# guanjq/targetdiff

Measured on AMD Instinct MI355X. Metric: ligands/sec (1000-step sampling, 100 samples/pocket) at 1/2/4/8 MI355X, higher is better.
Workload: dtype f32

## Files before the change

targetdiff_amd/csrc/edge16.hip:

```cpp
#include <type_traits>

#include "td_device.h"
#include "td_internal.h"

typedef float floatx4_t __attribute__((ext_vector_type(4)));

__device__ __forceinline__ floatx4_t td_mfma16(float a, float b, floatx4_t c) {
    return __builtin_amdgcn_mfma_f32_16x16x4f32(a, b, c, 0, 0, 0);
}

typedef _Float16 half8_16 __attribute__((ext_vector_type(8)));
__device__ __forceinline__ floatx4_t td_mfma16h(uint4 a, uint4 b, floatx4_t c) {
    return __builtin_amdgcn_mfma_f32_16x16x32_f16(__builtin_bit_cast(half8_16, a), __builtin_bit_cast(half8_16, b), c, 0, 0, 0);
}
__device__ __forceinline__ void td_split_h2(float x, float y, unsigned &h1, unsigned &h2) {
    h1 = __builtin_bit_cast(unsigned, __builtin_amdgcn_cvt_pkrtz(x, y));
    asm("v_fma_mixlo_f16 %0, %1, -1.0, %2 op_sel_hi:[1,0,0]\n\t"
        "v_fma_mixhi_f16 %0, %1, -1.0, %3 op_sel:[1,0,0] op_sel_hi:[1,0,0]"
        : "=&v"(h2) : "v"(h1), "v"(x), "v"(y));
}
constexpr float TD_Z_SCALE = 32768.0f;
__device__ __forceinline__ void td_split_h2_scaled_x4(const float (&x)[4], const float (&y)[4], unsigned (&h1)[4], unsigned (&h2)[4]) {
    const float S = TD_Z_SCALE;
    asm("v_fma_mixlo_f16 %0, %8, %16, 0\n\t"
// ... 1945 lines not shown
            a.h[(size_t)i * TD_H + nout + 4] = hres1 + o1;
        }
    }
    if (a.trace) {
        td_trace_wave_end(a.trace, lane);
        __syncthreads();
        if (tid == 0) a.trace[8 * blockIdx.x + 1] = __builtin_amdgcn_s_memrealtime();
    }
}

constexpr int TD_GATE_WGS = 1024;
constexpr int G16_WAVES = 4;
constexpr int G16Q_U4 = e16q_cs_u4<1>();
constexpr size_t G16_LDS_BYTES = (size_t)G16Q_U4 * 16 + (size_t)3 * TD_H * sizeof(float);

__global__ __launch_bounds__(G16_WAVES * 64) void edge_gate16_kernel(TdGate gt, const float4 *__restrict__ x4,
                                                                     const int32_t *__restrict__ nbr, int64_t N,
                                                                     const int32_t *__restrict__ rows,
                                                                     const int32_t *__restrict__ count_ptr,
                                                                     const int32_t *__restrict__ chunk_node, float *__restrict__ ew) {
    extern __shared__ __attribute__((aligned(16))) float lds[];
    const uint4 *Rp = reinterpret_cast<const uint4 *>(lds);
    float *B0 = lds + G16Q_U4 * 4, *BET = B0 + TD_H, *W3 = BET + TD_H;
    const int tid = threadIdx.x, lane = tid & 63, wid = tid >> 6;
    const int lo = lane & 15, g = lane >> 4;
    {
        td_stage_pk4<1>(gt.R16q, lds, 1, tid, G16_WAVES * 64);
        for (int t = tid; t < 3 * TD_H; t += G16_WAVES * 64) {
            const int n = t & (TD_H - 1);
            B0[t] = t < TD_H ? gt.b0[n] : (t < 2 * TD_H ? gt.beta[n] : gt.w3[n]);
        }
    }
    float offj[5];
#pragma unroll
    for (int j = 0; j < 5; ++j) offj[j] = gt.offsets[5 * g + j];
    __syncthreads();
    int64_t begin, end;
    td_node_range16(N, count_ptr, begin, end);
    const float c2 = gt.coeff * TD_LOG2E;

    for (int64_t it = begin + wid; it < end; it += G16_WAVES) {
        const int64_t row = rows ? (int64_t)rows[it] : it;
        const int64_t i = chunk_node ? (int64_t)chunk_node[row] : row;
        const float4 xi = x4[i];
        int jn[2];
        jn[0] = nbr[row * TD_K + lo];
        jn[1] = nbr[row * TD_K + 16 + lo];
        floatx4_t acc[2][8];
        uint4 bq[2][4];
        bool valid[2];
#pragma unroll
        for (int eb = 0; eb < 2; ++eb) {
            valid[eb] = jn[eb] >= 0;
            const float4 xj = x4[valid[eb] ? jn[eb] : (int)i];
            const float rx = xi.x - xj.x, ry = xi.y - xj.y, rz = xi.z - xj.z;
            const float dist = td_sqrt_d2(rx * rx + ry * ry + rz * rz);
            float gv[5];
#pragma unroll
            for (int j = 0; j < 5; ++j) {
                const float u = dist - offj[j];
                gv[j] = __builtin_amdgcn_exp2f(c2 * (u * u));
            }
            td_pk4_bquads(gv, 0u, bq[eb]);
#pragma unroll
            for (int hb = 0; hb < 8; ++hb) {
                const float4 b = *reinterpret_cast<const float4 *>(B0 + 16 * hb + 4 * g);
                acc[eb][hb][0] = b.x; acc[eb][hb][1] = b.y; acc[eb][hb][2] = b.z; acc[eb][hb][3] = b.w;
            }
        }
        td_pk4_tiles<1, 1, 2>(Rp + lane, lane, bq, acc);
        td_ln_relu16<2>(BET, g, acc, TdLn{gt.ln_c1, gt.ln_c2});
#pragma unroll
        for (int eb = 0; eb < 2; ++eb) {
            float part = 0.f;
#pragma unroll
            for (int hb = 0; hb < 8; ++hb) {
                const float4 w = *reinterpret_cast<const float4 *>(W3 + 16 * hb + 4 * g);
                part = fmaf(acc[eb][hb][0], w.x, part); part = fmaf(acc[eb][hb][1], w.y, part);
                part = fmaf(acc[eb][hb][2], w.z, part); part = fmaf(acc[eb][hb][3], w.w, part);
            }
            const float logit = td_sum_groups(part) + gt.b3;
            if (g == 0) ew[row * TD_K + 16 * eb + lo] = valid[eb] ? 1.0f / (1.0f + expf(-logit)) : 0.f;
        }
    }
}

template __global__ void edge_key16_kernel<false, K16S_WAVES, 0, 2, true, 0, 1>(Args16);
template __global__ void edge_key16_kernel<false, K16S_WAVES, 0, 2, true, 0, 0>(Args16);
template __global__ void edge_key16_kernel<false, K16S_WAVES, 0, 2, true, 2, 1>(Args16);
template __global__ void edge_key16_kernel<false, K16S_WAVES, 0, 2, true, 2, 0>(Args16);
template __global__ void edge_key16_kernel<false, K16S_WAVES, 0, 2, true, 1, 1>(Args16);
template __global__ void edge_key16_kernel<false, K16S_WAVES, 0, 2, true, 1, 0>(Args16);
template __global__ void edge_key16_kernel<false, K16S_WAVES, 0, 1, true, 0, 1>(Args16);
template __global__ void edge_key16_kernel<false, K16S_WAVES, 0, 1, true, 0, 0>(Args16);
template __global__ void edge_key16_kernel<false, K16S_WAVES, 0, 1, true, 2, 1>(Args16);
template __global__ void edge_key16_kernel<false, K16S_WAVES, 0, 1, true, 1, 1>(Args16);
template __global__ void edge_key16_kernel<false, K16S_WAVES, 1, 1, true, 0, 1>(Args16);
template __global__ void edge_key16_kernel<false, K16S_WAVES, 1, 1, true, 0, 0>(Args16);
template __global__ void edge_key16_kernel<false, K16S_WAVES, 1, 0, true, 0, 1>(Args16);
template __global__ void edge_key16_kernel<false, K16S_WAVES, 1, 0, true, 0, 0>(Args16);
// ... 219 lines not shown
    const bool split = mlp_k.use_split && mlp_v.use_split;
    if (cptr) {
        if (f16_first) return td_launch<edge_h2x16_chunked_kernel<1>>(grid, block, h2x16_lds_bytes<true>(), s, ar);
        return td_launch<edge_h2x16_chunked_kernel<0>>(grid, block, h2x16_lds_bytes<true>(), s, ar);
    }
    if (split && f16_first) return td_launch<edge_h2x16_kernel<true, 1>>(grid, block, h2x16_lds_bytes<true>(), s, ar);
    if (split) return td_launch<edge_h2x16_kernel<true, 0>>(grid, block, h2x16_lds_bytes<true>(), s, ar);
    return td_launch<edge_h2x16_kernel<false, 0>>(grid, block, h2x16_lds_bytes<false>(), s, ar);
}

int td_launch_gate16(const TdGate &g, const float4 *x4, const int32_t *nbr, int64_t N, const int32_t *rows,
                     const int32_t *count_ptr, float *ew, hipStream_t s, const int32_t *chunk_node) {
    if (N == 0) return TD_OK;
    int64_t G = (N + G16_WAVES - 1) / G16_WAVES;
    if (G > TD_GATE_WGS) G = TD_GATE_WGS;
    return td_launch<edge_gate16_kernel>(dim3((unsigned)G), dim3(G16_WAVES * 64), G16_LDS_BYTES, s, g, x4, nbr, N, rows, count_ptr, chunk_node, ew);
}
```

targetdiff_amd/csrc/graph.hip:

```cpp
#include "td_device.h"
#include "td_internal.h"

__global__ void graph_ptr_kernel(const int64_t *__restrict__ batch, int64_t N, int64_t B, int32_t *__restrict__ ptr) {
    int64_t i = (int64_t)blockIdx.x * blockDim.x + threadIdx.x;
    if (N == 0) {
        if (i <= B) ptr[i] = 0;
        return;
    }
    if (i >= N) return;
    int64_t b = batch[i];
    int64_t prev = (i == 0) ? -1 : batch[i - 1];
    for (int64_t g = prev + 1; g <= b && g <= B; ++g) ptr[g] = (int32_t)i;
    if (i == N - 1)
        for (int64_t g = b + 1; g <= B; ++g) ptr[g] = (int32_t)N;
}

int td_launch_graph_ptr(const int64_t *batch, int64_t N, int64_t B, int32_t *ptr, hipStream_t s) {
    int64_t n = N > B + 1 ? N : B + 1;
    graph_ptr_kernel<<<dim3((unsigned)((n + 255) / 256)), dim3(256), 0, s>>>(batch, N, B, ptr);
    TD_CHECK_HIP(hipGetLastError());
    return TD_OK;
}

__global__ void node_gid_kernel(const int32_t *__restrict__ ptr, int64_t N, int B, int32_t *__restrict__ gid) {
// ... 147 lines not shown
int td_launch_knn_rows(const float4 *x4, const int32_t *node_ptr, const int32_t *gid, const int32_t *rows, int64_t count,
                       int max_graph_nodes, int32_t *nbr, hipStream_t s, int k) {
    return launch_knn_t<false>(x4, node_ptr, gid, rows, count, max_graph_nodes, k, nbr, nullptr, s);
}

int td_launch_knn_static(const float4 *x4, const int32_t *node_ptr, const int32_t *gid, const int32_t *rows, int64_t count,
                         int max_graph_nodes, int32_t *nbr, unsigned long long *skeys, hipStream_t s, int k) {
    return launch_knn_t<true>(x4, node_ptr, gid, rows, count, max_graph_nodes, k, nbr, skeys, s);
}

struct TdMergeArgs {
    const float4 *x4; const int32_t *ptr, *pptr, *gid, *prot_rows; int64_t Np;
    const unsigned long long *skeys; const int32_t *snbr; const float *h0, *h1s, *ews; int32_t *nbr; float *h, *ew;
    uint8_t *clean, *flags2; int k;
    const int32_t *cgraph, *cbase;
};
__device__ __forceinline__ void knn_merge_body(unsigned bid, const TdMergeArgs &ma) {
    const float4 *__restrict__ x4 = ma.x4;
    const int32_t *__restrict__ ptr = ma.ptr, *__restrict__ pptr = ma.pptr, *__restrict__ gid = ma.gid, *__restrict__ prot_rows = ma.prot_rows;
    const int64_t Np = ma.Np;
    const unsigned long long *__restrict__ skeys = ma.skeys;
    const int32_t *__restrict__ snbr = ma.snbr;
    const float *__restrict__ h0 = ma.h0, *__restrict__ h1s = ma.h1s, *__restrict__ ews = ma.ews;
    int32_t *__restrict__ nbr = ma.nbr;
    float *__restrict__ h = ma.h, *__restrict__ ew = ma.ew;
    uint8_t *__restrict__ clean = ma.clean, *__restrict__ flags2 = ma.flags2;
    const int k = ma.k;
    const int lane = threadIdx.x & 63;
    const int64_t qi = (int64_t)bid * 4 + (threadIdx.x >> 6);
    if (qi >= Np) return;
// ... 1 lines not shown
    const int g = gid[i];
    const int lbeg = ptr[g] + (pptr[g + 1] - pptr[g]), lend = ptr[g + 1];
    const float4 xi = x4[i];
    int64_t c = i;
    int rebase = 0;
    if (ma.cgraph) {
        rebase = ptr[g] - ptr[ma.cgraph[g]];
        c = (int64_t)ma.cbase[g] + (i - ptr[g]);
    }
    unsigned long long ks = lane < TD_K ? skeys[c * TD_K + lane] : TD_KEY_MAX;
    if (ks != TD_KEY_MAX) ks += (unsigned long long)(unsigned)rebase;
    const unsigned long long thr = __shfl(ks, k - 1);
    unsigned long long kl[2] = {TD_KEY_MAX, TD_KEY_MAX};
    bool closer = false;
    bool overflow = lend - lbeg > 128;
#pragma unroll
    for (int u = 0; u < 2; ++u) {
        const int j = lbeg + lane + 64 * u;
        if (j < lend) {
            const float4 xj = x4[j];
            const float d2 = td_dist2(xj.x - xi.x, xj.y - xi.y, xj.z - xi.z);
            kl[u] = ((unsigned long long)__float_as_uint(d2) << 32) | (unsigned)j;
            closer |= kl[u] < thr;
        }
    }
    bool is_clean = !overflow && __ballot(closer) == 0ull;
    if (!is_clean && !overflow) {
        const bool c0 = kl[0] < thr, c1 = kl[1] < thr;
        const unsigned long long m0 = __ballot(c0), m1 = __ballot(c1);
        const int n_static = __popcll(__ballot(lane < TD_K && ks != TD_KEY_MAX));
// ... 1 lines not shown
        bool lig_in = false;
#pragma unroll
        for (int u = 0; u < 2; ++u) {
            unsigned long long mm = u ? m1 : m0;
            while (mm) {
                const int src = __builtin_amdgcn_readfirstlane(__ffsll((long long)mm) - 1);
                mm &= mm - 1;
                const unsigned clo = __builtin_amdgcn_readlane((int)(unsigned)kl[u], src);
                const unsigned chi = __builtin_amdgcn_readlane((int)(unsigned)(kl[u] >> 32), src);
                const unsigned long long ck = ((unsigned long long)chi << 32) | clo;
                if (lane < TD_K && ck < ks) ++shift;
                const int rank = __popcll(__ballot(lane < TD_K && ks < ck)) + __popcll(__ballot(c0 && kl[0] < ck)) +
                                 __popcll(__ballot(c1 && kl[1] < ck));
                if (rank < k) {
                    lig_in = true;
                    if (lane == 0) nbr[i * TD_K + rank] = (int32_t)clo;
                }
            }
        }
        const int total = n_static + __popcll(m0) + __popcll(m1);
        if (lane < TD_K) {
            const int pos = lane + shift;
            if (ks != TD_KEY_MAX && pos < k) nbr[i * TD_K + pos] = (int32_t)(unsigned)(ks & 0xffffffffull);
            if (lane >= (total < k ? total : k)) nbr[i * TD_K + lane] = -1;
        }
        is_clean = !lig_in;
    } else if (!is_clean) {
        unsigned long long best = ks;
        for (int base = lbeg; base < lend; base += 128) {
            if (base != lbeg) {
#pragma unroll
                for (int u = 0; u < 2; ++u) {
                    const int j = base + lane + 64 * u;
                    kl[u] = TD_KEY_MAX;
                    if (j < lend) {
                        const float4 xj = x4[j];
                        const float d2 = td_dist2(xj.x - xi.x, xj.y - xi.y, xj.z - xi.z);
                        kl[u] = ((unsigned long long)__float_as_uint(d2) << 32) | (unsigned)j;
                    }
                }
            }
// ... 13 lines not shown
            best = out;
        }
        if (lane < TD_K) nbr[i * TD_K + lane] = (best == TD_KEY_MAX || lane >= k) ? -1 : (int32_t)(unsigned)(best & 0xffffffffull);
        const bool lig_in = lane < k && best != TD_KEY_MAX && (int)(unsigned)(best & 0xffffffffull) >= lbeg;
        is_clean = __ballot(lig_in) == 0ull;
    } else if (lane < TD_K) {
        const int32_t sj = snbr[c * TD_K + lane];
        nbr[i * TD_K + lane] = sj >= 0 ? sj + rebase : -1;
    }
    const float2 hv = *reinterpret_cast<const float2 *>((is_clean ? h1s : h0) + c * TD_H + 2 * lane);
    *reinterpret_cast<float2 *>(h + i * TD_H + 2 * lane) = hv;
    if (is_clean && lane < TD_K) ew[i * TD_K + lane] = ews[c * TD_K + lane];
    if (lane == 0) {
        clean[i] = is_clean ? 1 : 0;
        if (flags2) flags2[i] = 0;
    }
}

__global__ __launch_bounds__(256) void knn_merge_kernel(TdMergeArgs ma) { knn_merge_body(blockIdx.x, ma); }

template <int CH>
__global__ __launch_bounds__(256) void knn_step_kernel(TdMergeArgs ma, unsigned GB, const int32_t *__restrict__ lig_rows, int64_t Nl,
                                                       int32_t *__restrict__ nbr) {
    if (blockIdx.x < GB) knn_body<CH, false>(blockIdx.x, ma.x4, ma.ptr, ma.gid, lig_rows, Nl, ma.k, nbr, nullptr);
    else knn_merge_body(blockIdx.x - GB, ma);
}

int td_launch_knn_merge(const float4 *x4, const int32_t *node_ptr, const int32_t *pptr, const int32_t *gid,
                        const int32_t *prot_rows, int64_t Np, const unsigned long long *skeys, const int32_t *snbr,
                        const float *h0, const float *h1s, const float *ews, int32_t *nbr, float *h, float *ew,
                        uint8_t *clean, uint8_t *flags2, hipStream_t s, int k, const int32_t *lig_rows, int64_t Nl,
                        int max_graph_nodes, const int32_t *cgraph, const int32_t *cbase) {
    const TdMergeArgs ma{x4, node_ptr, pptr, gid, prot_rows, Np, skeys, snbr, h0, h1s, ews, nbr, h, ew, clean, flags2, k, cgraph, cbase};
    const unsigned GA = (unsigned)((Np + 3) / 4), GB = lig_rows ? (unsigned)((Nl + 3) / 4) : 0u;
    if (GA + GB == 0) return TD_OK;
    if (GB == 0) {
        knn_merge_kernel<<<dim3(GA), dim3(256), 0, s>>>(ma);
    } else {
        const dim3 grid(GA + GB), block(256);
        if (max_graph_nodes > 0 && max_graph_nodes <= 256) knn_step_kernel<4><<<grid, block, 0, s>>>(ma, GB, lig_rows, Nl, nbr);
        else if (max_graph_nodes > 0 && max_graph_nodes <= 384) knn_step_kernel<6><<<grid, block, 0, s>>>(ma, GB, lig_rows, Nl, nbr);
        else if (max_graph_nodes <= 704) knn_step_kernel<11><<<grid, block, 0, s>>>(ma, GB, lig_rows, Nl, nbr);
        else knn_step_kernel<17><<<grid, block, 0, s>>>(ma, GB, lig_rows, Nl, nbr);
    }
    TD_CHECK_HIP(hipGetLastError());
    return TD_OK;
}

// ... 325 lines not shown
        int32_t *c = counter[0];
#pragma unroll
        for (int q = 1; q < L; ++q) c = l == q ? counter[q] : c;
        s_base[l] = (total && c) ? atomicAdd(c, total) : 0;
    }
    __syncthreads();
#pragma unroll
    for (int l = 0; l < L; ++l) {
        int before = 0;
        for (int w = 0; w < wave; ++w) before += s_cnt[l][w];
        slot[l] = s_base[l] + before + __popcll(m[l] & below);
    }
    __syncthreads();
}

constexpr int TD_LISTS_THREADS = 1024;

template <bool CHUNKED>
__global__ __launch_bounds__(TD_LISTS_THREADS) void step_lists_kernel(const uint8_t *__restrict__ clean, const float4 *__restrict__ x4,
                                                                      const int32_t *__restrict__ nbr, const int32_t *__restrict__ node_ptr,
                                                                      const int32_t *__restrict__ cptr, const int32_t *__restrict__ chunk_node,
                                                                      int64_t N, int cap, TdStepLists out) {
    constexpr int T = TD_LISTS_THREADS, RPT = T / TD_K;
    extern __shared__ uint8_t s_flags[];
    uint8_t *dirty = s_flags, *reach = s_flags + cap, *level = s_flags + 2 * cap, *lig = s_flags + 3 * cap;
    const int n0 = node_ptr[blockIdx.x], n = node_ptr[blockIdx.x + 1] - n0;
    const int tid = threadIdx.x, e = tid & 31, r0 = tid >> 5;
    const int t0 = CHUNKED ? cptr[n0] : n0, nt = CHUNKED ? cptr[n0 + n] - t0 : n;
    for (int a = tid; a < n; a += T) {
        const bool l = x4[n0 + a].w > 0.5f;
// ... 46 lines not shown
        bool flag[TD_STEP_LISTS];
        flag[0] = in && dirty[a];
        flag[1] = in && out.reach_rows && reach[a];
        flag[2] = in && out.reach_rows && !reach[a];
#pragma unroll
        for (int k = 0; k < TD_HOP_LEVELS; ++k) flag[3 + k] = k < out.levels && lv != 0 && lv <= k + 1;
        int slot[TD_STEP_LISTS];
        td_block_slots_each<TD_STEP_LISTS, T / 64>(flag, counters, slot);
        const int32_t i = n0 + a;
        if (flag[0]) out.dirty_rows[slot[0]] = i;
        if (flag[1]) out.reach_rows[slot[1]] = i;
        if (flag[2]) out.rest_rows[slot[2]] = i;
#pragma unroll
        for (int k = 0; k < TD_HOP_LEVELS; ++k)
            if (flag[3 + k]) out.level_rows[(size_t)k * N + slot[3 + k]] = i;
    }
    if (CHUNKED && out.dirty_chunks) {
        int32_t *const cc[1] = {out.dirty_chunk_count};
        for (int base = 0; base < nt; base += T) {
            const int t = base + tid;
            const bool flag[1] = {t < nt && dirty[dst_of(t < nt ? t : 0)]};
            int slot[1];
            td_block_slots_each<1, T / 64>(flag, cc, slot);
            if (flag[0]) out.dirty_chunks[slot[0]] = t0 + t;
        }
    }
}

int td_launch_step_lists(const uint8_t *clean, const float4 *x4, const int32_t *nbr, const int32_t *node_ptr, int64_t N,
                         int64_t B, int max_nodes, const TdStepLists &out, hipStream_t s, const int32_t *cptr,
// ... 8 lines not shown
        step_lists_kernel<false><<<dim3((unsigned)B), dim3(TD_LISTS_THREADS), bytes, s>>>(clean, x4, nbr, node_ptr, nullptr, nullptr, N, cap, out);
    TD_CHECK_HIP(hipGetLastError());
    return TD_OK;
}

__global__ __launch_bounds__(128) void ligand_update_kernel(const float *__restrict__ lpos, const int64_t *__restrict__ lv,
                                                            const int32_t *__restrict__ lig_node, int64_t Nl, int C,
                                                            const float *__restrict__ WlT, const float *__restrict__ bl,
                                                            float *__restrict__ h, float4 *__restrict__ x4, TdStepReset rs,
                                                            const float *__restrict__ gbias, const int32_t *__restrict__ gid) {
    const int n = threadIdx.x;
    if (blockIdx.x == 0) {
        if (rs.c0 && n < rs.n0) rs.c0[n] = 0;
        if (rs.c1 && n < rs.n1) rs.c1[n] = 0;
        if (rs.c2 && n < rs.n2) rs.c2[n] = 0;
    }
    const int64_t a0 = (int64_t)blockIdx.x * TD_COMPOSE_ATOMS;
    const float bias = bl[n];
    for (int a = 0; a < TD_COMPOSE_ATOMS; ++a) {
        const int64_t at = a0 + a;
        if (at >= Nl) break;
        const int64_t p = lig_node[at];
        int v = (int)lv[at];
        v = v < 0 ? 0 : (v >= C ? C - 1 : v);
        h[p * TD_H + n] = (gbias ? WlT[v * TD_H + n] + gbias[(size_t)gid[p] * TD_H + n] : WlT[v * TD_H + n]) + bias;
        if (n == 0) {
            x4[p] = make_float4(lpos[3 * at], lpos[3 * at + 1], lpos[3 * at + 2], 1.f);
            if (rs.flags2) rs.flags2[p] = 0;
        }
    }
// ... 307 lines not shown
```

targetdiff_amd/csrc/pack.cpp:

```cpp
#include <algorithm>
#include <atomic>
#include <cmath>
#include <cstdarg>
#include <cstdio>
#include <cstdlib>
#include <cstring>
#include <mutex>
#include <new>
#include <vector>

#include "td_device.h"
#include "td_internal.h"
#include "td_api.h"

using namespace tdapi;

namespace tdapi {



struct FoldedMlp {
    std::vector<float> w0, b0, g, b, w3, b3v;
    const float *b3;
    float ln_c1 = 1.f / 128.f, ln_c2 = 1e-5f;
// ... 353 lines not shown
enum OptKind { OPT_FLAG, OPT_CLAMPED, OPT_RANGED };
struct OptRow { const char *name; int TdOptions::*field; OptKind kind; int lo, hi; };
const OptRow OPTIONS[] = {
    {"h2x_fused", &TdOptions::h2x_fused, OPT_FLAG, 0, 1},
    {"node_proj_split", &TdOptions::node_proj_split, OPT_FLAG, 0, 1},
    {"node_proj_bpipe", &TdOptions::node_proj_bpipe, OPT_FLAG, 0, 1},
    {"node_proj_async", &TdOptions::node_proj_async, OPT_FLAG, 0, 1},
    {"edge_key_split", &TdOptions::edge_key_split, OPT_FLAG, 0, 1},
    {"edge_first_layer_f16", &TdOptions::edge_first_layer_f16, OPT_FLAG, 0, 1},
    {"edge_second_layer_f16", &TdOptions::edge_second_layer_f16, OPT_FLAG, 0, 1},
    {"edge_row_dealing", &TdOptions::edge_row_dealing, OPT_CLAMPED, 0, 2},
    {"session_hop_levels", &TdOptions::session_hop_levels, OPT_RANGED, 1, TD_HOP_LEVELS},
    {"session_forward_reach", &TdOptions::session_forward_reach, OPT_FLAG, 0, 1},
    {"session_step_lists", &TdOptions::session_step_lists, OPT_FLAG, 0, 1},
    {"session_share_pockets", &TdOptions::session_share_pockets, OPT_FLAG, 0, 1},
};
struct ReadOnlyRow { const char *name; int td_model::*field; };
const ReadOnlyRow READ_ONLY[] = {{"fold_dead_units", &td_model::fold_dead_units}, {"fold_fp32_mlps", &td_model::fold_fp32_mlps}};

template <class Row, size_t N>
const Row *find_row(const Row (&rows)[N], const char *name) {
    for (const Row &r : rows)
        if (strcmp(r.name, name) == 0) return &r;
    return nullptr;
}

void apply_options(td_model *m) {
    const TdOptions &o = m->opt;
    m->gate.use_split = o.edge_key_split != 0;
    for (int l = 0; l < m->cfg.num_layers * stage_rows(m->cfg); ++l) {
// ... 286 lines not shown
```

targetdiff_amd/csrc/session.cpp:

```cpp
#include <atomic>
#include <cmath>
#include <cstdarg>
#include <cstdio>
#include <cstdlib>
#include <cstring>
#include <map>
#include <mutex>
#include <new>
#include <vector>

#include "td_device.h"
#include "td_internal.h"
#include "td_api.h"

using namespace tdapi;

struct td_session {
    const td_model *m;
    int64_t N, Np, Nl, B;
    int max_graph_nodes;
    char *block;
    hipStream_t last_stream;
    Workspace w;
    int32_t *prot_node, *pptr, *lptr, *snbr, *dirty_rows, *dirty_count, *hop_rows, *hop_count, *dirty_chunks;
    int hop_levels;
    unsigned long long *skeys;
    float *ews, *h0, *h1s, *h2s, *P0, *q0;
    uint8_t *flags2;
    int32_t *fwd_rows, *fwd_rest, *fwd_counts;
    bool use_fwd;
    uint8_t *clean;
    float *setup_lpos; int64_t *setup_lv; int32_t *canon_rows;
    int graph_nodes_max;
    int32_t *cgraph = nullptr, *cbase = nullptr;
    int64_t static_rows = 0;
    int pocket_groups = 0;
    bool caching;
    bool chunked;
    GraphPlan plan;
    float *pred_pos, *pred_v;
    hipGraph_t graph;
    hipGraphExec_t graph_exec;
    td_step_io graph_io;
    unsigned graph_epoch = 0;
    int eager_steps;
    bool graph_failed, last_step_graph;
// ... 108 lines not shown
    S->prot_node = c.take<int32_t>(np);
    S->pptr = c.take<int32_t>(nb + 1); S->lptr = c.take<int32_t>(nb + 1);
    S->h0 = c.take<float>(ns * TD_H);
    S->setup_lpos = c.take<float>(nl * 3); S->setup_lv = c.take<int64_t>(nl);
    S->snbr = c.take<int32_t>(C * ncs * TD_K);
    S->skeys = c.take<unsigned long long>(C * ns * ks);
    S->ews = c.take<float>(C * ncs * TD_K);
    S->h1s = c.take<float>(C * ns * TD_H); S->h2s = c.take<float>(C * ns * TD_H);
    S->flags2 = c.take<uint8_t>(C * n);
    S->fwd_rows = c.take<int32_t>(C * n); S->fwd_rest = c.take<int32_t>(C * n); S->fwd_counts = c.take<int32_t>(64);
    S->P0 = c.take<float>(C * n * 4 * TD_H); S->q0 = c.take<float>(C * n * TD_H);
    S->clean = c.take<uint8_t>(C * n);
    S->dirty_rows = c.take<int32_t>(C * n); S->dirty_count = c.take<int32_t>(64);
    S->hop_rows = c.take<int32_t>(C * n * TD_HOP_LEVELS); S->hop_count = c.take<int32_t>(64);
    S->dirty_chunks = c.take<int32_t>(S->chunked ? C * nc : 0);
    S->pred_pos = c.take<float>(nl * 3); S->pred_v = c.take<float>(nl * TD_MAXC);
    S->cgraph = c.take<int32_t>(share ? nb : 0); S->cbase = c.take<int32_t>(share ? nb : 0);
    S->canon_rows = c.take<int32_t>(share ? ns : 0);
    if (!share) S->cgraph = S->cbase = S->canon_rows = nullptr;
    return S->w.bytes + c.off;
}

int session_build_static(td_session *S, const float *d_protein_pos, const float *d_protein_v, const int32_t *d_protein_ptr,
                         const int32_t *d_ligand_ptr, const PocketGroups &pg, hipStream_t s) {
    const td_model *m = S->m;
    const int64_t N = S->N, N_p = S->Np, N_l = S->Nl, B = S->B;
    const size_t n = (size_t)N, nb = (size_t)B;
    const bool share = S->cgraph != nullptr;
    Workspace &w = S->w;
    int rc;
// ... 73 lines not shown
extern "C" int td_session_create(const td_model *m, const float *d_protein_pos, const float *d_protein_v,
                                 const int32_t *d_protein_ptr, int64_t N_p, const int32_t *d_ligand_ptr, int64_t N_l,
                                 int64_t B, int32_t max_graph_nodes, void *stream, td_session **out) {
    if (!m || !out || N_p <= 0 || N_l <= 0 || B <= 0 || !d_protein_pos || !d_protein_v || !d_protein_ptr || !d_ligand_ptr) {
        td_set_error("td_session_create: bad argument");
        return TD_EINVAL;
    }
    hipStream_t s = static_cast<hipStream_t>(stream);
    td_session *S = new (std::nothrow) td_session();
    if (!S) { td_set_error("td_session_create: out of host memory"); return TD_ENOMEM; }
    SessionGuard guard{S, s};
    S->m = m; S->N = N_p + N_l; S->Np = N_p; S->Nl = N_l; S->B = B; S->max_graph_nodes = max_graph_nodes; S->last_stream = s;
    int rc;
    std::vector<int32_t> hp, hl;
    if ((rc = fetch_ptrs(d_protein_ptr, d_ligand_ptr, B, hp, hl, s)) != TD_OK) return rc;
    int gmax = 0;
    for (int64_t g = 0; g < B; ++g) gmax = std::max(gmax, (hp[g + 1] - hp[g]) + (hl[g + 1] - hl[g]));
    S->graph_nodes_max = gmax;
    S->chunked = !default_graph(m->cfg);
    const bool knn_like = m->cfg.cutoff_mode == TD_CUTOFF_KNN || m->cfg.cutoff_mode == TD_CUTOFF_HYBRID;
    S->caching = knn_like && (!S->chunked || gmax <= TD_STEP_LISTS_MAX_NODES) && num_blocks(m->cfg) == 1 && m->cfg.ew_net_type == 0 &&
                 !m->cfg.x2h_out_fc && !m->cfg.sync_twoup && stage_rows(m->cfg) == 1;
    S->use_fwd = S->caching && m->opt.session_forward_reach && m->cfg.num_layers >= 2;
    S->hop_levels = std::min(std::min(std::max(m->opt.session_hop_levels, 1), TD_HOP_LEVELS), m->cfg.num_layers);
    if (S->chunked && (rc = plan_create(m->cfg, hp.data(), hl.data(), B, s, &S->plan)) != TD_OK) return rc;
    const bool share = S->caching && !S->chunked && m->opt.session_share_pockets != 0;
    PocketGroups pg;
    if (share) {
        if ((rc = group_pockets(m, d_protein_pos, d_protein_v, d_protein_ptr, B, hp, hl, s, &pg)) != TD_OK) return rc;
        S->static_rows = (int64_t)pg.canon_rows.size();
        S->pocket_groups = pg.groups;
    }
    const size_t bytes = session_layout(S, nullptr, share);
    hipError_t e = td_malloc_async(reinterpret_cast<void **>(&S->block), bytes, s);
    if (e != hipSuccess) { S->block = nullptr; td_set_error("td_session_create: hipMallocAsync(%zu) failed: %s", bytes, hipGetErrorString(e)); return TD_ENOMEM; }
    session_layout(S, S->block, share);
    if ((rc = session_build_static(S, d_protein_pos, d_protein_v, d_protein_ptr, d_ligand_ptr, pg, s)) != TD_OK) return rc;
// ... 28 lines not shown
            if ((rc = td_launch_ligand_update(m, d_ligand_pos, d_ligand_v, w.lig_node, Nl, w.h, w.x4a, s, nullptr, d_ligand_graph_bias, w.gid)) != TD_OK) return rc;
        }
        float4 *xg = nullptr;
        Workspace wb = w;
        if ((rc = run_blocks(m, wb, S->chunked ? &S->plan : nullptr, wb.h, N, Nl, 0, S->max_graph_nodes, &xg, s)) != TD_OK) return rc;
        ProfScope ps(PC_HEAD, s);
        return td_launch_head(m->head, w.h, xg, w.lig_node, Nl, m->cfg.ligand_num_classes, d_pred_ligand_pos, d_pred_ligand_v,
                              d_final_ligand_h, s);
    }
    {
        ProfScope ps(PC_COMPOSE, s);
        TdStepReset rs;
        rs.c0 = S->dirty_count; rs.n0 = 2;
        rs.c1 = S->fwd_counts; rs.n1 = 2;
        rs.c2 = S->hop_count; rs.n2 = TD_HOP_LEVELS;
        rs.flags2 = S->use_fwd ? S->flags2 : nullptr;
        if ((rc = td_launch_ligand_update(m, d_ligand_pos, d_ligand_v, w.lig_node, Nl, w.h, w.x4a, s, &rs, d_ligand_graph_bias, w.gid)) != TD_OK) return rc;
    }
    bool lists_done = false;
    {
        ProfScope ps(PC_KNN, s);
        const TdStepLists lists{S->dirty_rows, S->dirty_count, S->use_fwd ? S->fwd_rows : nullptr, S->fwd_rest, S->fwd_counts,
                                S->hop_rows, S->hop_count, S->hop_levels, S->chunked ? S->dirty_chunks : nullptr,
                                S->chunked ? S->dirty_count + 1 : nullptr};
        if (S->chunked) {
            const GraphPlan &p = S->plan;
            if ((rc = td_launch_knn_merge_general(w.x4a, w.node_ptr, S->pptr, w.gid, S->prot_node, Np, S->skeys, S->snbr, S->h0,
                                                  S->h1s, S->ews, p.cptr, p.cpn_p, p.cnbr, w.h, p.ew, S->clean,
                                                  S->use_fwd ? S->flags2 : nullptr, s, m->cfg.knn)) != TD_OK) return rc;
            if ((rc = td_launch_ligand_rows_general(p.mode, w.x4a, w.node_ptr, S->pptr, w.gid, w.lig_node, Nl, p.k, S->graph_nodes_max,
                                                    p.cptr, p.cnbr, s)) != TD_OK) return rc;
            if ((rc = td_launch_step_lists(S->clean, w.x4a, p.cnbr, w.node_ptr, N, S->B, S->graph_nodes_max, lists, s, p.cptr,
                                           p.chunk_node)) != TD_OK) {
                if (rc == TD_EINVAL) td_set_error("td_session_forward: a graph of %d nodes does not fit the row-list kernel", S->graph_nodes_max);
                return rc;
            }
            lists_done = true;
        } else {
            if ((rc = td_launch_knn_merge(w.x4a, w.node_ptr, S->pptr, w.gid, S->prot_node, Np, S->skeys, S->snbr, S->h0,
                                          S->h1s, S->ews, w.nbr, w.h, w.ew, S->clean, S->use_fwd ? S->flags2 : nullptr, s, m->cfg.knn,
                                          w.lig_node, Nl, S->max_graph_nodes, S->cgraph, S->cbase)) != TD_OK) return rc;
            rc = (m->opt.session_step_lists && S->graph_nodes_max > 0) ? td_launch_step_lists(S->clean, w.x4a, w.nbr, w.node_ptr, N, S->B, S->graph_nodes_max, lists, s)
                                        : TD_EINVAL;
            lists_done = rc == TD_OK;
            if (rc != TD_OK && rc != TD_EINVAL) return rc;
            if (!lists_done) {
                if ((rc = td_launch_compact_dirty(S->clean, w.x4a, N, S->dirty_rows, S->dirty_count, s)) != TD_OK) return rc;
                if (S->use_fwd) {
                    if ((rc = td_launch_forward_reach(S->clean, w.x4a, w.nbr, N, S->flags2, S->fwd_rows, S->fwd_rest, S->fwd_counts,
                                                      S->clean, s)) != TD_OK) return rc;
                } else {
                    TD_CHECK_HIP(hipMemsetAsync(S->clean, 0, (size_t)N, s));
                }
            }
        }
    }
    {
        ProfScope ps(PC_GATE, s);
        if (S->chunked)
            rc = td_launch_gate(m->gate, w.x4a, gt.nbr, S->plan.NC, S->dirty_chunks, S->dirty_count + 1, gt.ew, s, S->plan.chunk_node);
        else
            rc = td_launch_gate(m->gate, w.x4a, gt.nbr, N, S->dirty_rows, S->dirty_count, gt.ew, s);
        if (rc != TD_OK) return rc;
    }
    {
        X2hStage a;
        a.P = S->P0; a.q = S->q0; a.lig = w.lig_node; a.Nl = Nl;
        a.proj = RowSel{w.lig_node, nullptr, Nl};
        a.rows = RowSel{S->dirty_rows, S->dirty_count, N};
        if ((rc = x2h_stage(m->layers[0], gt, w.x4a, w.h, N, a, s)) != TD_OK) return rc;
    }
    if (!lists_done && (rc = td_launch_hop_levels(w.lig_node, Nl, w.nbr, N, S->clean, S->hop_rows, S->hop_count, S->hop_levels, s, true)) != TD_OK) return rc;
    float4 *xf = nullptr;
    const FwdReach fwd{S->fwd_rows, S->fwd_rest, S->fwd_counts, S->h2s, S->cbase};
    CachedStep cs;
// ... 178 lines not shown
```

targetdiff_amd/csrc/td_internal.h:

```cpp
#pragma once

#include <hip/hip_runtime.h>
#include <stddef.h>
#include <stdint.h>

#include <atomic>
#include <type_traits>

#include "../../include/targetdiff_hip.h"

constexpr int TD_H = 128;
constexpr int TD_HEADS = 16;
constexpr int TD_DH = 8;
constexpr int TD_K = 32;
constexpr int TD_NG = 20;
constexpr int TD_SLOTK = 24;
constexpr int TD_SLOT_STEPS = TD_SLOTK / 2;
constexpr int TD_KSTEPS = TD_H / 2;
constexpr int TD_MAXC = 16;
constexpr int TD_SMALL_BATCH_ROWS = 16384;

void td_set_error(const char *fmt, ...);
#define TD_CHECK_HIP(expr)                                                                       \
    do {                                                                                         \
// ... 130 lines not shown
};

struct TdOptions {
    int h2x_fused = 1;
    int node_proj_split = 1;
    int edge_key_split = 1;
    int edge_first_layer_f16 = 1;
    int edge_second_layer_f16 = 1;
    int session_hop_levels = 4;
    int session_forward_reach = 1;
    int edge_row_dealing = 2;
    int node_proj_bpipe = 0;
    int node_proj_async = 1;
    int session_share_pockets = 1;
    int session_step_lists = 1;
};

struct td_model {
    td_config cfg;
    TdOptions opt;
    float *blob;
    size_t blob_floats;
    TdEmbed emb;
    TdGate gate;
    TdLayer *layers;
    TdHead head;
    TdSchedules sched;
    unsigned option_epoch = 0;
    int fold_dead_units = 0;
    int fold_fp32_mlps = 0;
// ... 5 lines not shown
int td_launch_unpack_x(const float4 *x4, int64_t N, float *x3, hipStream_t s);
int td_launch_knn(const float4 *x4, const int32_t *node_ptr, const int32_t *gid, int64_t N, int max_graph_nodes,
                  int32_t *nbr, hipStream_t s, int k = TD_K);
int td_launch_compose(const td_model *m, const float *ppos, const float *pv, const int32_t *pptr, int64_t Np,
                      const float *lpos, const int64_t *lv, const int32_t *lptr, int64_t Nl, int64_t B,
                      float *h, float4 *x4, int32_t *node_ptr, int32_t *gid, int32_t *lig_node, int32_t *prot_node,
                      hipStream_t s, const float *gbias = nullptr);
int td_launch_knn_rows(const float4 *x4, const int32_t *node_ptr, const int32_t *gid, const int32_t *rows, int64_t count,
                       int max_graph_nodes, int32_t *nbr, hipStream_t s, int k = TD_K);
int td_launch_knn_static(const float4 *x4, const int32_t *node_ptr, const int32_t *gid, const int32_t *rows, int64_t count,
                         int max_graph_nodes, int32_t *nbr, unsigned long long *skeys, hipStream_t s, int k = TD_K);
int td_launch_knn_merge(const float4 *x4, const int32_t *node_ptr, const int32_t *pptr, const int32_t *gid,
                        const int32_t *prot_rows, int64_t Np, const unsigned long long *skeys, const int32_t *snbr,
                        const float *h0, const float *h1s, const float *ews, int32_t *nbr, float *h, float *ew,
                        uint8_t *clean, uint8_t *flags2, hipStream_t s, int k = TD_K, const int32_t *lig_rows = nullptr, int64_t Nl = 0,
                        int max_graph_nodes = 0, const int32_t *cgraph = nullptr, const int32_t *cbase = nullptr);
int td_launch_pocket_hash(const float *ppos, const float *pv, const int32_t *pptr, int64_t B, int F, unsigned long long *out, hipStream_t s);
int td_launch_pocket_verify(const float *ppos, const float *pv, const int32_t *pptr, int64_t B, int F, const int32_t *cand, int32_t *flags,
                            hipStream_t s);
int td_launch_compact_rows(const void *src, const int32_t *rows, int64_t n_rows, int row_bytes, void *dst, hipStream_t s);
int td_launch_compact_dirty(const uint8_t *clean, const float4 *x4, int64_t N, int32_t *rows, int32_t *count,
                            hipStream_t s);
int td_launch_forward_reach(const uint8_t *clean, const float4 *x4, const int32_t *nbr, int64_t N, uint8_t *flags2,
                            int32_t *rows_on, int32_t *rows_off, int32_t *counts2, uint8_t *clean_to_zero, hipStream_t s);
int td_launch_restore_rows(const int32_t *rows, const int32_t *count_ptr, int64_t max_rows, const float *hs, float *h,
                           hipStream_t s, const int32_t *gid = nullptr, const int32_t *node_ptr = nullptr, const int32_t *cbase = nullptr);
constexpr int TD_HOP_LEVELS = 4;
int td_launch_hop_levels(const int32_t *lig_node, int64_t Nl, const int32_t *nbr, int64_t N, uint8_t *flags,
                         int32_t *rows, int32_t *counts, int levels, hipStream_t s, bool zeroed = false);
int td_launch_gate16(const TdGate &g, const float4 *x4, const int32_t *nbr, int64_t N, const int32_t *rows,
                     const int32_t *count_ptr, float *ew, hipStream_t s, const int32_t *chunk_node);
struct TdStepLists {
    int32_t *dirty_rows, *dirty_count;
    int32_t *reach_rows, *rest_rows, *reach_counts;
    int32_t *level_rows, *level_counts;
    int levels;
    int32_t *dirty_chunks = nullptr, *dirty_chunk_count = nullptr;
};
int td_launch_step_lists(const uint8_t *clean, const float4 *x4, const int32_t *nbr, const int32_t *node_ptr, int64_t N,
                         int64_t B, int max_nodes, const TdStepLists &out, hipStream_t s, const int32_t *cptr = nullptr,
                         const int32_t *chunk_node = nullptr);
struct TdStepReset {
    int32_t *c0 = nullptr, *c1 = nullptr, *c2 = nullptr;
    int n0 = 0, n1 = 0, n2 = 0;
    uint8_t *flags2 = nullptr;
};
int td_launch_ligand_update(const td_model *m, const float *lpos, const int64_t *lv, const int32_t *lig_node, int64_t Nl,
                            float *h, float4 *x4, hipStream_t s, const TdStepReset *reset = nullptr, const float *gbias = nullptr,
                            const int32_t *gid = nullptr);
int td_launch_ligand_list(const uint8_t *mask, int64_t N, int32_t *lig_node, int32_t *count, hipStream_t s);
int td_launch_node_proj(const TdNodeStage &st, const float *h, int64_t N, const int32_t *rows, unsigned mat_mask,
                        float *P, float *q, hipStream_t s, const int32_t *count_ptr = nullptr,
                        const int32_t *rows2 = nullptr, int64_t N2 = 0, unsigned mask2 = 0);
int td_launch_node_proj_pair(const TdNodeStage &hx, const int32_t *hop_rows, const int32_t *hop_count,
                             const int32_t *lig_rows, int64_t Nl, float *Px, float *qx, const TdNodeStage &nx,
                             const int32_t *rows, const int32_t *count_ptr, float *P, float *q, const float *h, int64_t N,
                             hipStream_t s);
int td_launch_node_output(const TdNodeOut &no, const float *out, float *h, int64_t N, hipStream_t s);
int td_launch_layer_gate(const float *w, const float *offsets, float coeff, const float4 *x4, const int32_t *nbr, int64_t N, float *ew,
// ... 269 lines not shown
```

Measured before the change: 26.95.

## Gate only ligand-touched edges instead of every edge of dirty rows

The kNN merge now records which neighbor slots of each protein node point at ligand atoms, and it copies cached edge weights for the other slots. The step-lists kernel compacts those ligand slots into an edge list, and a templated gate kernel evaluates the edge MLP only on ligand rows plus those listed edges. Previously every edge of every dirty row was recomputed. This adds a bitmask buffer, a block-level prefix-sum allocation and extra writes in the merge, and it is enabled by default under eligibility conditions.

```diff
diff --git a/targetdiff_amd/csrc/edge16.hip b/targetdiff_amd/csrc/edge16.hip
--- a/targetdiff_amd/csrc/edge16.hip
+++ b/targetdiff_amd/csrc/edge16.hip
@@ -1983,11 +1983,14 @@
 constexpr int G16Q_U4 = e16q_cs_u4<1>();
 constexpr size_t G16_LDS_BYTES = (size_t)G16Q_U4 * 16 + (size_t)3 * TD_H * sizeof(float);
 
+template <bool EDGES>
 __global__ __launch_bounds__(G16_WAVES * 64) void edge_gate16_kernel(TdGate gt, const float4 *__restrict__ x4,
                                                                      const int32_t *__restrict__ nbr, int64_t N,
                                                                      const int32_t *__restrict__ rows,
                                                                      const int32_t *__restrict__ count_ptr,
-                                                                     const int32_t *__restrict__ chunk_node, float *__restrict__ ew) {
+                                                                     const int32_t *__restrict__ chunk_node, float *__restrict__ ew,
+                                                                     const int32_t *__restrict__ edges,
+                                                                     const int32_t *__restrict__ edge_count) {
     extern __shared__ __attribute__((aligned(16))) float lds[];
     const uint4 *Rp = reinterpret_cast<const uint4 *>(lds);
     float *B0 = lds + G16Q_U4 * 4, *BET = B0 + TD_H, *W3 = BET + TD_H;
@@ -2005,21 +2008,36 @@
     for (int j = 0; j < 5; ++j) offj[j] = gt.offsets[5 * g + j];
     __syncthreads();
     int64_t begin, end;
-    td_node_range16(N, count_ptr, begin, end);
+    const int64_t n_edges = EDGES ? (int64_t)*edge_count : 0;
+    if (EDGES) td_node_range16(N + (n_edges + TD_K - 1) / TD_K, nullptr, begin, end);
+    else td_node_range16(N, count_ptr, begin, end);
     const float c2 = gt.coeff * TD_LOG2E;
 
     for (int64_t it = begin + wid; it < end; it += G16_WAVES) {
-        const int64_t row = rows ? (int64_t)rows[it] : it;
-        const int64_t i = chunk_node ? (int64_t)chunk_node[row] : row;
-        const float4 xi = x4[i];
+        int64_t slot[2], ie[2];
+        if (EDGES && it >= N) {
+#pragma unroll
+            for (int eb = 0; eb < 2; ++eb) {
+                const int64_t rec = (it - N) * TD_K + 16 * eb + lo;
+                slot[eb] = rec < n_edges ? (int64_t)edges[rec] : -1;
+                ie[eb] = slot[eb] < 0 ? 0 : slot[eb] / TD_K;
+            }
+        } else {
+            const int64_t row = rows ? (int64_t)rows[it] : it;
+            slot[0] = row * TD_K + lo;
+            slot[1] = row * TD_K + 16 + lo;
+            ie[0] = ie[1] = chunk_node ? (int64_t)chunk_node[row] : row;
+        }
         int jn[2];
-        jn[0] = nbr[row * TD_K + lo];
-        jn[1] = nbr[row * TD_K + 16 + lo];
+        jn[0] = slot[0] < 0 ? -1 : nbr[slot[0]];
+        jn[1] = slot[1] < 0 ? -1 : nbr[slot[1]];
         floatx4_t acc[2][8];
         uint4 bq[2][4];
         bool valid[2];
 #pragma unroll
         for (int eb = 0; eb < 2; ++eb) {
+            const int64_t i = ie[eb];
+            const float4 xi = x4[i];
             valid[eb] = jn[eb] >= 0;
             const float4 xj = x4[valid[eb] ? jn[eb] : (int)i];
             const float rx = xi.x - xj.x, ry = xi.y - xj.y, rz = xi.z - xj.z;
@@ -2049,10 +2067,12 @@
                 part = fmaf(acc[eb][hb][2], w.z, part); part = fmaf(acc[eb][hb][3], w.w, part);
             }
             const float logit = td_sum_groups(part) + gt.b3;
-            if (g == 0) ew[row * TD_K + 16 * eb + lo] = valid[eb] ? 1.0f / (1.0f + expf(-logit)) : 0.f;
-        }
-    }
-}
+            if (g == 0 && slot[eb] >= 0) ew[slot[eb]] = valid[eb] ? 1.0f / (1.0f + expf(-logit)) : 0.f;
+        }
+    }
+}
+template __global__ void edge_gate16_kernel<false>(TdGate, const float4 *, const int32_t *, int64_t, const int32_t *, const int32_t *, const int32_t *,
+                                                   float *, const int32_t *, const int32_t *);
 
 template __global__ void edge_key16_kernel<false, K16S_WAVES, 0, 2, true, 0, 1>(Args16);
 template __global__ void edge_key16_kernel<false, K16S_WAVES, 0, 2, true, 0, 0>(Args16);
@@ -2302,5 +2322,16 @@
     if (N == 0) return TD_OK;
     int64_t G = (N + G16_WAVES - 1) / G16_WAVES;
     if (G > TD_GATE_WGS) G = TD_GATE_WGS;
-    return td_launch<edge_gate16_kernel>(dim3((unsigned)G), dim3(G16_WAVES * 64), G16_LDS_BYTES, s, g, x4, nbr, N, rows, count_ptr, chunk_node, ew);
-}
+    return td_launch<edge_gate16_kernel<false>>(dim3((unsigned)G), dim3(G16_WAVES * 64), G16_LDS_BYTES, s, g, x4, nbr, N, rows, count_ptr, chunk_node, ew,
+                                                nullptr, nullptr);
+}
+
+int td_launch_gate16_edges(const TdGate &g, const float4 *x4, const int32_t *nbr, const int32_t *rows, int64_t n_rows, const int32_t *edges,
+                           const int32_t *edge_count, int64_t max_edges, float *ew, hipStream_t s) {
+    const int64_t most = n_rows + (max_edges + TD_K - 1) / TD_K;
+    if (most == 0) return TD_OK;
+    int64_t G = (most + G16_WAVES - 1) / G16_WAVES;
+    if (G > TD_GATE_WGS) G = TD_GATE_WGS;
+    return td_launch<edge_gate16_kernel<true>>(dim3((unsigned)G), dim3(G16_WAVES * 64), G16_LDS_BYTES, s, g, x4, nbr, n_rows, rows, nullptr, nullptr, ew,
+                                               edges, edge_count);
+}
diff --git a/targetdiff_amd/csrc/graph.hip b/targetdiff_amd/csrc/graph.hip
--- a/targetdiff_amd/csrc/graph.hip
+++ b/targetdiff_amd/csrc/graph.hip
@@ -185,6 +185,7 @@
     const unsigned long long *skeys; const int32_t *snbr; const float *h0, *h1s, *ews; int32_t *nbr; float *h, *ew;
     uint8_t *clean, *flags2; int k;
     const int32_t *cgraph, *cbase;
+    uint32_t *lig_slots;
 };
 __device__ __forceinline__ void knn_merge_body(unsigned bid, const TdMergeArgs &ma) {
     const float4 *__restrict__ x4 = ma.x4;
@@ -216,6 +217,7 @@
     unsigned long long kl[2] = {TD_KEY_MAX, TD_KEY_MAX};
     bool closer = false;
     bool overflow = lend - lbeg > 128;
+    unsigned lig_slots = 0;
 #pragma unroll
     for (int u = 0; u < 2; ++u) {
         const int j = lbeg + lane + 64 * u;
@@ -247,6 +249,7 @@
                                  __popcll(__ballot(c1 && kl[1] < ck));
                 if (rank < k) {
                     lig_in = true;
+                    lig_slots |= 1u << rank;
                     if (lane == 0) nbr[i * TD_K + rank] = (int32_t)clo;
                 }
             }
@@ -254,10 +257,17 @@
         const int total = n_static + __popcll(m0) + __popcll(m1);
         if (lane < TD_K) {
             const int pos = lane + shift;
-            if (ks != TD_KEY_MAX && pos < k) nbr[i * TD_K + pos] = (int32_t)(unsigned)(ks & 0xffffffffull);
-            if (lane >= (total < k ? total : k)) nbr[i * TD_K + lane] = -1;
+            if (ks != TD_KEY_MAX && pos < k) {
+                nbr[i * TD_K + pos] = (int32_t)(unsigned)(ks & 0xffffffffull);
+                if (ma.lig_slots) ew[i * TD_K + pos] = ews[c * TD_K + lane];
+            }
+            if (lane >= (total < k ? total : k)) {
+                nbr[i * TD_K + lane] = -1;
+                if (ma.lig_slots) ew[i * TD_K + lane] = 0.f;
+            }
         }
         is_clean = !lig_in;
+        if (is_clean) lig_slots = 0;
     } else if (!is_clean) {
         unsigned long long best = ks;
         for (int base = lbeg; base < lend; base += 128) {
@@ -301,6 +311,7 @@
     if (lane == 0) {
         clean[i] = is_clean ? 1 : 0;
         if (flags2) flags2[i] = 0;
+        if (ma.lig_slots) ma.lig_slots[i] = lig_slots;
     }
 }
 
@@ -317,8 +328,9 @@
                         const int32_t *prot_rows, int64_t Np, const unsigned long long *skeys, const int32_t *snbr,
                         const float *h0, const float *h1s, const float *ews, int32_t *nbr, float *h, float *ew,
                         uint8_t *clean, uint8_t *flags2, hipStream_t s, int k, const int32_t *lig_rows, int64_t Nl,
-                        int max_graph_nodes, const int32_t *cgraph, const int32_t *cbase) {
-    const TdMergeArgs ma{x4, node_ptr, pptr, gid, prot_rows, Np, skeys, snbr, h0, h1s, ews, nbr, h, ew, clean, flags2, k, cgraph, cbase};
+                        int max_graph_nodes, const int32_t *cgraph, const int32_t *cbase, uint32_t *lig_slots) {
+    const TdMergeArgs ma{x4, node_ptr, pptr, gid, prot_rows, Np, skeys, snbr, h0, h1s, ews, nbr, h, ew, clean, flags2, k, cgraph, cbase,
+                         lig_slots};
     const unsigned GA = (unsigned)((Np + 3) / 4), GB = lig_rows ? (unsigned)((Nl + 3) / 4) : 0u;
     if (GA + GB == 0) return TD_OK;
     if (GB == 0) {
@@ -674,6 +686,32 @@
     __syncthreads();
 }
 
+template <int WAVES>
+__device__ __forceinline__ int td_block_slots_weighted(int w, int32_t *counter) {
+    __shared__ int s_cnt[WAVES];
+    __shared__ int s_base;
+    const int lane = threadIdx.x & 63, wave = threadIdx.x >> 6;
+    int inc = w;
+#pragma unroll
+    for (int d = 1; d < 64; d <<= 1) {
+        const int below = __shfl_up(inc, d);
+        if (lane >= d) inc += below;
+    }
+    if (lane == 63) s_cnt[wave] = inc;
+    __syncthreads();
+    if (threadIdx.x == 0) {
+        int total = 0;
+        for (int q = 0; q < WAVES; ++q) total += s_cnt[q];
+        s_base = total ? atomicAdd(counter, total) : 0;
+    }
+    __syncthreads();
+    int before = 0;
+    for (int q = 0; q < wave; ++q) before += s_cnt[q];
+    const int first = s_base + before + inc - w;
+    __syncthreads();
+    return first;
+}
+
 constexpr int TD_LISTS_THREADS = 1024;
 
 template <bool CHUNKED>
@@ -750,6 +788,11 @@
 #pragma unroll
         for (int k = 0; k < TD_HOP_LEVELS; ++k)
             if (flag[3 + k]) out.level_rows[(size_t)k * N + slot[3 + k]] = i;
+        if (!CHUNKED && out.edges) {
+            const unsigned m = (in && !lig[a]) ? out.lig_slots[i] : 0u;
+            int at = td_block_slots_weighted<T / 64>(__popc(m), out.edge_count);
+            for (unsigned mm = m; mm; mm &= mm - 1u) out.edges[at++] = i * TD_K + (__ffs((int)mm) - 1);
+        }
     }
     if (CHUNKED && out.dirty_chunks) {
         int32_t *const cc[1] = {out.dirty_chunk_count};
@@ -788,6 +831,7 @@
         if (rs.c0 && n < rs.n0) rs.c0[n] = 0;
         if (rs.c1 && n < rs.n1) rs.c1[n] = 0;
         if (rs.c2 && n < rs.n2) rs.c2[n] = 0;
+        if (rs.c3 && n < rs.n3) rs.c3[n] = 0;
     }
     const int64_t a0 = (int64_t)blockIdx.x * TD_COMPOSE_ATOMS;
     const float bias = bl[n];
diff --git a/targetdiff_amd/csrc/pack.cpp b/targetdiff_amd/csrc/pack.cpp
--- a/targetdiff_amd/csrc/pack.cpp
+++ b/targetdiff_amd/csrc/pack.cpp
@@ -391,6 +391,7 @@
     {"session_forward_reach", &TdOptions::session_forward_reach, OPT_FLAG, 0, 1},
     {"session_step_lists", &TdOptions::session_step_lists, OPT_FLAG, 0, 1},
     {"session_share_pockets", &TdOptions::session_share_pockets, OPT_FLAG, 0, 1},
+    {"session_edge_gate", &TdOptions::session_edge_gate, OPT_FLAG, 0, 1},
 };
 struct ReadOnlyRow { const char *name; int td_model::*field; };
 const ReadOnlyRow READ_ONLY[] = {{"fold_dead_units", &td_model::fold_dead_units}, {"fold_fp32_mlps", &td_model::fold_fp32_mlps}};
diff --git a/targetdiff_amd/csrc/session.cpp b/targetdiff_amd/csrc/session.cpp
--- a/targetdiff_amd/csrc/session.cpp
+++ b/targetdiff_amd/csrc/session.cpp
@@ -30,6 +30,9 @@
     int32_t *fwd_rows, *fwd_rest, *fwd_counts;
     bool use_fwd;
     uint8_t *clean;
+    uint32_t *lig_slots = nullptr;
+    int32_t *gate_edges = nullptr, *gate_edge_count = nullptr;
+    bool edge_gate = false;
     float *setup_lpos; int64_t *setup_lv; int32_t *canon_rows;
     int graph_nodes_max;
     int32_t *cgraph = nullptr, *cbase = nullptr;
@@ -168,6 +171,9 @@
     S->dirty_rows = c.take<int32_t>(C * n); S->dirty_count = c.take<int32_t>(64);
     S->hop_rows = c.take<int32_t>(C * n * TD_HOP_LEVELS); S->hop_count = c.take<int32_t>(64);
     S->dirty_chunks = c.take<int32_t>(S->chunked ? C * nc : 0);
+    const size_t E = S->edge_gate ? 1 : 0;
+    S->lig_slots = c.take<uint32_t>(E * n); S->gate_edges = c.take<int32_t>(E * np * TD_K); S->gate_edge_count = c.take<int32_t>(E * 64);
+    if (!S->edge_gate) { S->lig_slots = nullptr; S->gate_edges = S->gate_edge_count = nullptr; }
     S->pred_pos = c.take<float>(nl * 3); S->pred_v = c.take<float>(nl * TD_MAXC);
     S->cgraph = c.take<int32_t>(share ? nb : 0); S->cbase = c.take<int32_t>(share ? nb : 0);
     S->canon_rows = c.take<int32_t>(share ? ns : 0);
@@ -271,13 +277,17 @@
     int rc;
     std::vector<int32_t> hp, hl;
     if ((rc = fetch_ptrs(d_protein_ptr, d_ligand_ptr, B, hp, hl, s)) != TD_OK) return rc;
-    int gmax = 0;
-    for (int64_t g = 0; g < B; ++g) gmax = std::max(gmax, (hp[g + 1] - hp[g]) + (hl[g + 1] - hl[g]));
+    int gmax = 0, lmax = 0;
+    for (int64_t g = 0; g < B; ++g) {
+        gmax = std::max(gmax, (hp[g + 1] - hp[g]) + (hl[g + 1] - hl[g]));
+        lmax = std::max(lmax, hl[g + 1] - hl[g]);
+    }
     S->graph_nodes_max = gmax;
     S->chunked = !default_graph(m->cfg);
     const bool knn_like = m->cfg.cutoff_mode == TD_CUTOFF_KNN || m->cfg.cutoff_mode == TD_CUTOFF_HYBRID;
     S->caching = knn_like && (!S->chunked || gmax <= TD_STEP_LISTS_MAX_NODES) && num_blocks(m->cfg) == 1 && m->cfg.ew_net_type == 0 &&
                  !m->cfg.x2h_out_fc && !m->cfg.sync_twoup && stage_rows(m->cfg) == 1;
+    S->edge_gate = S->caching && !S->chunked && lmax <= 128 && gmax > 0 && gmax <= TD_STEP_LISTS_MAX_NODES && S->N < (int64_t(1) << 26);
     S->use_fwd = S->caching && m->opt.session_forward_reach && m->cfg.num_layers >= 2;
     S->hop_levels = std::min(std::min(std::max(m->opt.session_hop_levels, 1), TD_HOP_LEVELS), m->cfg.num_layers);
     if (S->chunked && (rc = plan_create(m->cfg, hp.data(), hl.data(), B, s, &S->plan)) != TD_OK) return rc;
@@ -336,15 +346,18 @@
         rs.c0 = S->dirty_count; rs.n0 = 2;
         rs.c1 = S->fwd_counts; rs.n1 = 2;
         rs.c2 = S->hop_count; rs.n2 = TD_HOP_LEVELS;
+        rs.c3 = S->gate_edge_count; rs.n3 = S->gate_edge_count ? 1 : 0;
         rs.flags2 = S->use_fwd ? S->flags2 : nullptr;
         if ((rc = td_launch_ligand_update(m, d_ligand_pos, d_ligand_v, w.lig_node, Nl, w.h, w.x4a, s, &rs, d_ligand_graph_bias, w.gid)) != TD_OK) return rc;
     }
     bool lists_done = false;
+    const bool edge_gate = S->edge_gate && m->opt.session_edge_gate != 0 && m->opt.session_step_lists != 0 && m->gate.use_split;
     {
         ProfScope ps(PC_KNN, s);
-        const TdStepLists lists{S->dirty_rows, S->dirty_count, S->use_fwd ? S->fwd_rows : nullptr, S->fwd_rest, S->fwd_counts,
-                                S->hop_rows, S->hop_count, S->hop_levels, S->chunked ? S->dirty_chunks : nullptr,
-                                S->chunked ? S->dirty_count + 1 : nullptr};
+        TdStepLists lists{S->dirty_rows, S->dirty_count, S->use_fwd ? S->fwd_rows : nullptr, S->fwd_rest, S->fwd_counts,
+                          S->hop_rows, S->hop_count, S->hop_levels, S->chunked ? S->dirty_chunks : nullptr,
+                          S->chunked ? S->dirty_count + 1 : nullptr};
+        if (edge_gate) { lists.lig_slots = S->lig_slots; lists.edges = S->gate_edges; lists.edge_count = S->gate_edge_count; }
         if (S->chunked) {
             const GraphPlan &p = S->plan;
             if ((rc = td_launch_knn_merge_general(w.x4a, w.node_ptr, S->pptr, w.gid, S->prot_node, Np, S->skeys, S->snbr, S->h0,
@@ -361,7 +374,7 @@
         } else {
             if ((rc = td_launch_knn_merge(w.x4a, w.node_ptr, S->pptr, w.gid, S->prot_node, Np, S->skeys, S->snbr, S->h0,
                                           S->h1s, S->ews, w.nbr, w.h, w.ew, S->clean, S->use_fwd ? S->flags2 : nullptr, s, m->cfg.knn,
-                                          w.lig_node, Nl, S->max_graph_nodes, S->cgraph, S->cbase)) != TD_OK) return rc;
+                                          w.lig_node, Nl, S->max_graph_nodes, S->cgraph, S->cbase, edge_gate ? S->lig_slots : nullptr)) != TD_OK) return rc;
             rc = (m->opt.session_step_lists && S->graph_nodes_max > 0) ? td_launch_step_lists(S->clean, w.x4a, w.nbr, w.node_ptr, N, S->B, S->graph_nodes_max, lists, s)
                                         : TD_EINVAL;
             lists_done = rc == TD_OK;
@@ -381,6 +394,8 @@
         ProfScope ps(PC_GATE, s);
         if (S->chunked)
             rc = td_launch_gate(m->gate, w.x4a, gt.nbr, S->plan.NC, S->dirty_chunks, S->dirty_count + 1, gt.ew, s, S->plan.chunk_node);
+        else if (edge_gate && lists_done)
+            rc = td_launch_gate16_edges(m->gate, w.x4a, gt.nbr, w.lig_node, Nl, S->gate_edges, S->gate_edge_count, Np * TD_K, gt.ew, s);
         else
             rc = td_launch_gate(m->gate, w.x4a, gt.nbr, N, S->dirty_rows, S->dirty_count, gt.ew, s);
         if (rc != TD_OK) return rc;
diff --git a/targetdiff_amd/csrc/td_internal.h b/targetdiff_amd/csrc/td_internal.h
--- a/targetdiff_amd/csrc/td_internal.h
+++ b/targetdiff_amd/csrc/td_internal.h
@@ -168,6 +168,7 @@
     int node_proj_async = 1;
     int session_share_pockets = 1;
     int session_step_lists = 1;
+    int session_edge_gate = 1;
 };
 
 struct td_model {
@@ -203,7 +204,8 @@
                         const int32_t *prot_rows, int64_t Np, const unsigned long long *skeys, const int32_t *snbr,
                         const float *h0, const float *h1s, const float *ews, int32_t *nbr, float *h, float *ew,
                         uint8_t *clean, uint8_t *flags2, hipStream_t s, int k = TD_K, const int32_t *lig_rows = nullptr, int64_t Nl = 0,
-                        int max_graph_nodes = 0, const int32_t *cgraph = nullptr, const int32_t *cbase = nullptr);
+                        int max_graph_nodes = 0, const int32_t *cgraph = nullptr, const int32_t *cbase = nullptr,
+                        uint32_t *lig_slots = nullptr);
 int td_launch_pocket_hash(const float *ppos, const float *pv, const int32_t *pptr, int64_t B, int F, unsigned long long *out, hipStream_t s);
 int td_launch_pocket_verify(const float *ppos, const float *pv, const int32_t *pptr, int64_t B, int F, const int32_t *cand, int32_t *flags,
                             hipStream_t s);
@@ -219,19 +221,23 @@
                          int32_t *rows, int32_t *counts, int levels, hipStream_t s, bool zeroed = false);
 int td_launch_gate16(const TdGate &g, const float4 *x4, const int32_t *nbr, int64_t N, const int32_t *rows,
                      const int32_t *count_ptr, float *ew, hipStream_t s, const int32_t *chunk_node);
+int td_launch_gate16_edges(const TdGate &g, const float4 *x4, const int32_t *nbr, const int32_t *rows, int64_t n_rows, const int32_t *edges,
+                           const int32_t *edge_count, int64_t max_edges, float *ew, hipStream_t s);
 struct TdStepLists {
     int32_t *dirty_rows, *dirty_count;
     int32_t *reach_rows, *rest_rows, *reach_counts;
     int32_t *level_rows, *level_counts;
     int levels;
     int32_t *dirty_chunks = nullptr, *dirty_chunk_count = nullptr;
+    const uint32_t *lig_slots = nullptr;
+    int32_t *edges = nullptr, *edge_count = nullptr;
 };
 int td_launch_step_lists(const uint8_t *clean, const float4 *x4, const int32_t *nbr, const int32_t *node_ptr, int64_t N,
                          int64_t B, int max_nodes, const TdStepLists &out, hipStream_t s, const int32_t *cptr = nullptr,
                          const int32_t *chunk_node = nullptr);
 struct TdStepReset {
-    int32_t *c0 = nullptr, *c1 = nullptr, *c2 = nullptr;
-    int n0 = 0, n1 = 0, n2 = 0;
+    int32_t *c0 = nullptr, *c1 = nullptr, *c2 = nullptr, *c3 = nullptr;
+    int n0 = 0, n1 = 0, n2 = 0, n3 = 0;
     uint8_t *flags2 = nullptr;
 };
 int td_launch_ligand_update(const td_model *m, const float *lpos, const int64_t *lv, const int32_t *lig_node, int64_t Nl,
```

After: 27.18 (median of 6 runs). About the same (+0.9%).
